# mx-mark/VideoTransformer-pytorch

Hardware: AMD Instinct MI355X
Metric: clips/sec TimeSformer-B divided_space_time 8x3x224x224 fwd+bwd (whole job) (higher is better)
Workload: dtype bf16

## Files before the change

videotransformer-pytorch_amd/csrc/gemm_nt.hip:

```cpp
#include "gemm_common.h"

namespace vtx {

constexpr int BK16 = 64;

__global__ __launch_bounds__(NT_THREADS) void gemm_nt_bf16_kernel(
    int M, int N, int K, const bf16raw* __restrict__ A, long lda, vtx_rowmap amap,
    const bf16raw* __restrict__ B, long ldb, int tiles_n, EpiParams ep) {
  extern __shared__ __attribute__((aligned(16))) char smem[];
  bf16raw* As = reinterpret_cast<bf16raw*>(smem);
  bf16raw* Bs = As + 2 * BM * BK16;
  const int tid = threadIdx.x, lane = tid & 63, wave = tid >> 6;
  const int wm = wave >> 1, wn = wave & 1;
  const int nwg = gridDim.x;
  const int tile = xcd_remap(blockIdx.x, nwg);
  const int tm = tile / tiles_n, tn = tile - tm * tiles_n;
  const int m0 = tm * BM, n0 = tn * BN;

  const int lc = tid & 7, lr = tid >> 3;
  const bf16raw* ap[4];
  const bf16raw* bp[4];
  int lds_off[4];
#pragma unroll
  for (int it = 0; it < 4; ++it) {
// ... 374 lines not shown
    asm volatile("" : "+v"(lq));
#pragma unroll
    for (int j = 0; j < 2; ++j) {
      const int rho = (wave * 2 + j) * 8 + (lq >> 3);
      const unsigned c2 = (unsigned)(((lq & 7) ^ ((rho >> 1) & 7)) * 16);
      const int la0 = min((rho >> 6) * 128 + (rho & 63), ml), la1 = min((rho >> 6) * 128 + (rho & 63) + 64, ml);
      const int lb0 = min((rho >> 5) * 64 + (rho & 31), nl), lb1 = min((rho >> 5) * 64 + (rho & 31) + 32, nl);
      unsigned ra0, ra1;
      if (CONT || am.fast) {
        ra0 = (unsigned)(la0 + (la0 >= bl ? am.skip : 0));
        ra1 = (unsigned)(la1 + (la1 >= bl ? am.skip : 0));
      } else {
        ra0 = (unsigned)(map_row(amap, m0s + la0) - first);
        ra1 = (unsigned)(map_row(amap, m0s + la1) - first);
      }
      off[0][j] = ra0 * lda2 + c2;
      off[3][j] = ra1 * lda2 + c2;
      off[1][j] = (unsigned)lb0 * ldb2 + c2;
      off[2][j] = (unsigned)lb1 * ldb2 + c2;
    }
  };
  auto issue = [&](int kind, int kt) {
    bf16raw* dst = lds + ((kt & 1) ^ par) * PP_BUF + kind * PP_REGION + wave * 1024;
    const char* base = ((kind == 0 || kind == 3) ? abase : bbase) + (long)kt * (PP_BK * 2);
    asm volatile("" : "+s"(base));
    dma16(reinterpret_cast<const bf16raw*>(base + off[kind][0]), dst);
    dma16(reinterpret_cast<const bf16raw*>(base + off[kind][1]), dst + 512);
  };
  auto prologue = [&]() {
    issue(0, 0); issue(1, 0); issue(2, 0); issue(3, 0);
    issue(0, 1); issue(1, 1); issue(2, 1);
  };

  const int l31 = lane & 31;
  int fr[4];
#pragma unroll
  for (int ks = 0; ks < 4; ++ks) fr[ks] = l31 * PP_BK + (((2 * ks + (lane >> 5)) ^ ((l31 >> 1) & 7)) << 3);
  const int a_grp = wr * 64 * PP_BK;
  const int b_grp = wc * 32 * PP_BK;

#define PP_READ_A(buf_, kind_)                                                                         \
  _Pragma("unroll") for (int i = 0; i < 2; ++i) _Pragma("unroll") for (int ks = 0; ks < 4; ++ks)       \
      fa[i][ks] = *reinterpret_cast<const bf16x8*>(lds + (buf_) * PP_BUF + (kind_) * PP_REGION + a_grp + i * 32 * PP_BK + fr[ks]);
#define PP_READ_B(buf_, kind_, fb_)                                                                    \
  _Pragma("unroll") for (int ks = 0; ks < 4; ++ks)                                                     \
      fb_[ks] = *reinterpret_cast<const bf16x8*>(lds + (buf_) * PP_BUF + (kind_) * PP_REGION + b_grp + fr[ks]);
#define PP_MMA(i0_, j_, fb_, ISSUE_) PP_MMA_H(i0_, j_, fb_, ISSUE_, , )
#ifndef VTX_PP_PRIO
#define VTX_PP_PRIO 1
#endif
#define PP_MMA_H(i0_, j_, fb_, ISSUE_, HW_, HB_)                                                       \
  if (VTX_PP_PRIO == 1) __builtin_amdgcn_s_setprio(1); else if (VTX_PP_PRIO == 3) __builtin_amdgcn_s_setprio(0); \
  _Pragma("unroll") for (int ks = 0; ks < 4; ++ks) {                                                   \
    _Pragma("unroll") for (int i = 0; i < 2; ++i)                                                      \
        acc[(i0_) + i][j_] = __builtin_amdgcn_mfma_f32_32x32x16_bf16(fa[i][ks], fb_[ks], acc[(i0_) + i][j_], 0, 0, 0); \
    if (ks == 0) { __builtin_amdgcn_sched_barrier(0); ISSUE_; HW_ __builtin_amdgcn_sched_barrier(0); HB_ }     \
  }                                                                                                    \
  if (VTX_PP_PRIO == 1) __builtin_amdgcn_s_setprio(0); else if (VTX_PP_PRIO == 3) __builtin_amdgcn_s_setprio(1);
#define PP_BAR() __builtin_amdgcn_s_barrier()

#ifndef VTX_PP_BF16_STAGE
#define VTX_PP_BF16_STAGE 1
#endif
#define PP_KTILE(E1_, E2_, W1_, W2_, W4_, ISS_, H1_, H2_, H3_, H4_) PP_KTILE_X(E1_, E2_, W1_, W2_, W4_, ISS_, H1_, H2_, H3_, H4_, false, false, false)
#define PP_KTILE_X(E1_, E2_, W1_, W2_, W4_, ISS_, H1_, H2_, H3_, H4_, X1_, X2_, X4_) \
    PP_KTILE_XH(E1_, E2_, W1_, W2_, W4_, ISS_, H1_, H2_, H3_, H4_, X1_, X2_, X4_, false, false, , , , )
#define PP_KTILE_XH(E1_, E2_, W1_, W2_, W4_, ISS_, H1_, H2_, H3_, H4_, X1_, X2_, X4_, X1R_, R4_, M3W_, M3B_, M4W_, M4B_) \
    {                                                                                                  \
      const int buf = (kt & 1) ^ par;                                                                  \
      const bool e1 = (E1_), e2 = (E2_);                   \
      const bool w1 = (W1_), w2 = (W2_);            \
                                                            \
      PP_READ_A(buf, 0);                                                                               \
      PP_READ_B(buf, 1, fb0);                                                                          \
      if (w1) { if (X1_) { if (X1R_) wait_vmcnt<8 + NST - NSR>(); else wait_vmcnt<8 + NST>(); } else wait_vmcnt<8>(); } else wait_vmcnt<2>(); \
      H1_                                                                                              \
      lgkm0();                                                                                         \
      PP_BAR();                                                                                        \
      PP_MMA(0, 0, fb0, ISS_(3, kt + 1, e1));                                                          \
      PP_BAR();                                                                                        \
                                                                \
      PP_READ_B(buf, 2, fb1);                                                                          \
      if (w1) { if (X2_) wait_vmcnt<8 + NST>(); else wait_vmcnt<8>(); } else wait_vmcnt<0>();          \
      H2_                                                                                              \
      lgkm0();                                                                                         \
      PP_BAR();                                                                                        \
      PP_MMA(0, 1, fb1, ISS_(0, kt + 2, e2));                                                          \
      PP_BAR();                                                                                        \
                                                                                     \
      PP_READ_A(buf, 3);                                                                               \
      H3_                                                                                              \
      lgkm0();                                                                                         \
      PP_BAR();                                                                                        \
      PP_MMA_H(2, 1, fb1, ISS_(1, kt + 2, e2), M3W_, M3B_);                                            \
      PP_BAR();                                                                                        \
                                 \
      if (W4_) { if (w2) { if (X4_) wait_vmcnt<8 + NST>(); else if (R4_) wait_vmcnt<10>(); else wait_vmcnt<8>(); } else if (w1) wait_vmcnt<4>(); } \
      H4_                                                                                              \
      PP_BAR();                                                                                        \
      PP_MMA_H(2, 0, fb0, ISS_(2, kt + 2, e2), M4W_, M4B_);                                            \
      PP_BAR();                                                                                        \
    }
#define PP_ISS_COND(kind_, ktv_, ex_) if (ex_) issue(kind_, ktv_)
#define PP_ISS_ALWAYS(kind_, ktv_, ex_) issue(kind_, ktv_)

  typedef __attribute__((address_space(3))) char lds_char;
  const unsigned slot_rd = (unsigned)(unsigned long)(lds_char*)(smem + PP_RING_BYTES);
  const unsigned bias_rd = (unsigned)(unsigned long)(lds_char*)(reinterpret_cast<char*>(stg) + 256 + (lane & 31) * 4);
  constexpr int NST = HAS_ACT ? 32 : 16;
  constexpr int NSR = NST / 4;
  bool relax = false;
  bool prev_rolled = false;
  int t = next_tile();
  const int tend = xcount;
  if (t >= tend) { check_out(); return; }
  int t_next = tend, t_nn = tend;
  if constexpr (CONT) t_next = next_tile();
  int pending = 0;
  if (EPI2 && !CONT && tid == 0) pending = atomicAdd(my_ctr, 1);
  set_tile(t, 0);
  m0 = m0s; n0 = n0s;
  prologue();
  while (true) {
    f32x16 acc[4][2];
#pragma unroll
    for (int i = 0; i < 4; ++i)
#pragma unroll
      for (int j = 0; j < 2; ++j)
#pragma unroll
        for (int r = 0; r < 16; ++r) acc[i][j][r] = 0.f;
    bf16x8 fa[2][4], fb0[4], fb1[4];
    if constexpr (PREG) {
      int lf = lane;
      asm volatile("" : "+v"(lf));
#pragma unroll
      for (int ks = 0; ks < 4; ++ks) fr[ks] = (lf & 31) * PP_BK + (((2 * ks + (lf >> 5)) ^ (((lf & 31) >> 1) & 7)) << 3);
    }
    const bool more_c = CONT && t_next < tend;
    const int em0 = m0 + wr * 128, en0 = n0 + wc * 64;
    const int tile_m0 = m0;
    TileMap cm;
    unsigned ldcb = 0, lean_skipb = 0;
    bool lean = false;
    [[maybe_unused]] bool rolled = false;
    int lean_lb = 0;
    const char* lean_cb = nullptr;
    [[maybe_unused]] __amdgpu_buffer_rsrc_t lean_rsrc;
    float bcol[2] = {0.f, 0.f};
    auto epi_head = [&]() {
      cm = make_tile_map(ep.cmap, tile_m0);
      ldcb = (unsigned)ep.ldc * 2u;
      const long skipb64 = (long)cm.skip * (long)ldcb;
      lean = CONT && (dbg == 0 || dbg == 5 || dbg == 6) && em0 + 127 < ep.M && en0 + 63 < ep.N && (ep.split_row <= 0 || em0 + 127 < ep.split_row) &&
             cm.fast && cm.skip >= 0 && skipb64 < (1L << 30) && ep.ldc < (1L << 22) && PRE != PRE_DGELU;
      if constexpr (HAS_ACT) lean = lean && ep.act == 2 && ep.ldc2 < (1L << 22);
      if constexpr (ROLL) lean = true;
      lean_lb = em0 < cm.bound ? cm.bound - em0 : 0x7fffffff;
      lean_cb = reinterpret_cast<const char*>(ep.C) + ((cm.base_q + em0 + (em0 >= cm.bound ? (long)cm.skip : 0L)) * ep.ldc + en0) * 2;
      lean_skipb = (unsigned)skipb64;
      if constexpr (ROLL) {
        const long last = (long)ep.cmap.base + (ep.M - 1) + (ep.cmap.grp > 0 ? (long)((unsigned)(ep.M - 1) / (unsigned)ep.cmap.grp) * ep.cmap.skip : 0L);
        const long left = en0 < ep.N ? (reinterpret_cast<const char*>(ep.C) + (last + 1) * ep.ldc * 2) - lean_cb : 0L;
        lean_rsrc = __builtin_amdgcn_make_buffer_rsrc(const_cast<char*>(lean_cb), 0, (int)(left < 0 ? 0 : (left > 0x7fffffffL ? 0x7fffffffL : left)), 0x00020000);
      }
    };
    typedef __attribute__((ext_vector_type(2))) __bf16 bf16x2;
    [[maybe_unused]] unsigned pl_wa0 = 0, pl_wa1 = 0, pl_rd = 0, pl_v0 = 0;
    [[maybe_unused]] int pl_p2 = 0;
    [[maybe_unused]] u32x4 pl_w0, pl_w1;
    auto pl_setup = [&]() {
      int ln = lane;
      asm volatile("" : "+v"(ln));
      const unsigned stg0 = (unsigned)(unsigned long)(lds_char*)(reinterpret_cast<char*>(stg));
      pl_p2 = ln >> 3;
      pl_wa0 = stg0 + (unsigned)(((ln >> 5) * 132 + (ln & 31)) * 4);
      pl_wa1 = pl_wa0 + 264 * 4;
      pl_rd = stg0 + (unsigned)((pl_p2 * 64 + 4 * ((pl_p2 >> 1) & 1) + 8 * (pl_p2 >> 2) + (ln & 7) * 8) * 4);
      pl_v0 = (unsigned)(2 * pl_p2) * ldcb + (unsigned)(ln & 7) * 16u;
    };
#define PP_LWAIT(n_, ...) asm volatile("s_waitcnt lgkmcnt(%[cnt])" : __VA_ARGS__ : [cnt] "n"(n_) : "memory"); __builtin_amdgcn_sched_barrier(0)
#define PP_PWAIT(n_) PP_LWAIT(n_, "+v"(pl_w0), "+v"(pl_w1))
#define PP_PW(mi_, half_) if (ep.bias) { PP_PW_(mi_, half_, true) } else { PP_PW_(mi_, half_, false) }
#define PP_PW_(mi_, half_, B_)                                                                          \
    {                                                                                                   \
      _Pragma("unroll") for (int kk = 0; kk < 2; ++kk) _Pragma("unroll") for (int ni = 0; ni < 2; ++ni) { \
        f32x2 lo = mk2(acc[mi_][ni][8 * (half_) + 4 * kk], acc[mi_][ni][8 * (half_) + 4 * kk + 1]);     \
        f32x2 hi = mk2(acc[mi_][ni][8 * (half_) + 4 * kk + 2], acc[mi_][ni][8 * (half_) + 4 * kk + 3]); \
        if (B_) { const f32x2 b2 = mk2(bcol[ni], bcol[ni]); lo = lo + b2; hi = hi + b2; }               \
        union { bf16x2 v; unsigned u; } x;      \
        union { bf16x2 v; unsigned u; } y;      \
        x.v[0] = (__bf16)lo[0]; x.v[1] = (__bf16)lo[1];                                                 \
        y.v[0] = (__bf16)hi[0]; y.v[1] = (__bf16)hi[1];                                                 \
        if (ni == 0) asm volatile("ds_write2_b32 %0, %1, %2 offset1:64" :: "v"(kk ? pl_wa1 : pl_wa0), "v"(x.u), "v"(y.u) : "memory"); \
        else asm volatile("ds_write2_b32 %0, %1, %2 offset0:32 offset1:96" :: "v"(kk ? pl_wa1 : pl_wa0), "v"(x.u), "v"(y.u) : "memory"); \
      }                                                                                                 \
    }
#define PP_PR() asm volatile("ds_read_b128 %0, %2\n\tds_read_b128 %1, %2 offset:16" : "=&v"(pl_w0), "=&v"(pl_w1) : "v"(pl_rd) : "memory")
#define PP_PF(p_)                                                                                       \
    {                                                                                                   \
      const char* base = lean_cb + (long)(16 * (p_)) * ldcb;                                            \
      if constexpr (!ROLL) asm volatile("" : "+s"(base));            \
      _Pragma("unroll") for (int u = 0; u < 2; ++u) {                                                   \
        const unsigned sel = u ? 0x07060302u : 0x05040100u;                                             \
        u32x4 o;                                                                                        \
        o[0] = __builtin_amdgcn_perm(pl_w0[1], pl_w0[0], sel);                                          \
        o[1] = __builtin_amdgcn_perm(pl_w0[3], pl_w0[2], sel);                                          \
        o[2] = __builtin_amdgcn_perm(pl_w1[1], pl_w1[0], sel);                                          \
        o[3] = __builtin_amdgcn_perm(pl_w1[3], pl_w1[2], sel);                                          \
        const unsigned voff = pl_v0 + (u ? ldcb : 0u) + ((2 * pl_p2 + u >= lean_lb - 16 * (p_)) ? lean_skipb : 0u); \
         \
         \
        if constexpr (ROLL) __builtin_amdgcn_raw_buffer_store_b128(o, lean_rsrc, voff + (unsigned)(16 * (p_)) * ldcb, 0, 2); \
        else st16_nt_b(base, voff, o);                                                                  \
      }                                                                                                 \
    }
    constexpr bool ROLLK = ROLL;
    static_assert(!ROLL || (CONT && VTX_PP_BF16_STAGE && PRE == PRE_NONE && !HAS_SC && !HAS_ACT), "rolling: the plain continuous flow only");
    stamp(0);
    if (relax) wait_vmcnt<10 + NST>(); else wait_vmcnt<10>();
    PP_BAR();
    stamp(1);
    if (wr == 1) PP_BAR();
    if constexpr (CONT) {
      auto bias_dma = [&]() {
        if (ep.bias) {
          const int c = n0 + wc * 64 + lane;
          __builtin_amdgcn_global_load_lds((const __attribute__((address_space(1))) void*)(ep.bias + (c < ep.N ? c : 0)),
// ... 10 lines not shown
            const int idx = split ? (ml - ep.split_row) : (int)q1 * ep.rs_m1 + (ml - (int)q2 * ep.rs_d2) * ep.rs_m2;
            __builtin_amdgcn_global_load_lds((const __attribute__((address_space(1))) void*)(ep.row_scale + idx),
                                             (__attribute__((address_space(3))) void*)(stg + 128 + h * 64), 4, 0, 0);
          }
        }
      };
      int drawn;
      asm volatile("" : "=v"(drawn));
      const int one = 1;
      int kt = 0;
      if (more_c) {
#define PP_CF_H1 if (kt == 0) bias_dma();                                                                        \
                 if (kt == 1 && tid == 0)                                                                        \
                   asm volatile("global_atomic_add %0, %1, %2, off sc0" : "=&v"(drawn) : "v"(my_ctr), "v"(one) : "memory");
#define PP_CF_H2 if (kt == nk - 2) set_tile(t_next, (long)nk * (PP_BK * 2));
#define PP_CF_H3 if (kt == 2) {                                                                                  \
                   int v;                                                                                        \
                   asm volatile("ds_read_b32 %0, %1\n\ts_waitcnt lgkmcnt(0)" : "=&v"(v) : "v"(slot_rd) : "memory"); \
                   t_nn = __builtin_amdgcn_readfirstlane(v);                                                     \
                 }
#define PP_CF_H4 if (kt == 1 && wave == 0) {                                                                     \
                   wait_vmcnt<6>();                                                                              \
                   if (tid == 0) asm volatile("ds_write_b32 %0, %1" :: "v"(slot_rd), "v"(drawn) : "memory");     \
                   lgkm0();                                                                                      \
                 }
        for (; kt < nk - 1; ++kt) {
          PP_KTILE_XH(true, true, true, true, true, PP_ISS_ALWAYS, PP_CF_H1, PP_CF_H2;, PP_CF_H3, PP_CF_H4,
                      relax && kt < 2, relax && kt == 0, relax && kt == 0, prev_rolled && kt == 1, false, , , , )
        }
        if constexpr (ROLLK) {
          epi_head();
          rolled = true;
          const bool full = em0 + 127 < ep.M && en0 + 63 < ep.N && trace == nullptr;
          if (ep.bias) asm volatile("ds_read_b32 %0, %2\n\tds_read_b32 %1, %2 offset:128\n\ts_waitcnt lgkmcnt(0)"
                                    : "=&v"(bcol[0]), "=&v"(bcol[1]) : "v"(bias_rd) : "memory");
          pl_setup();
          PP_KTILE_XH(true, true, true, true, true, PP_ISS_ALWAYS, , , PP_PW(0, 0) PP_PR();,
                      PP_PWAIT(0); PP_PF(1) PP_PW(1, 0) PP_PR();,
                      false, false, false, false, full,
                      , PP_PF(0) PP_PW(0, 1) PP_PR();,
                      PP_PWAIT(0);, PP_PF(2) PP_PW(1, 1) PP_PR();)
        } else {
          PP_KTILE_XH(true, true, true, true, true, PP_ISS_ALWAYS, PP_CF_H1, PP_CF_H2;, PP_CF_H3, PP_CF_H4,
                      relax && kt < 2, relax && kt == 0, relax && kt == 0, prev_rolled && kt == 1, false, , , , )
        }
#undef PP_CF_H1
#undef PP_CF_H2
#undef PP_CF_H3
#undef PP_CF_H4
      } else {
        for (; kt < nk; ++kt) {
          PP_KTILE(kt + 1 < nk, kt + 2 < nk, kt + 1 < nk, kt + 2 < nk, true, PP_ISS_COND, if (kt == 0) bias_dma();, , , )
        }
      }
    } else {
      for (int kt = 0; kt < nk; ++kt) {
        PP_KTILE(kt + 1 < nk, kt + 2 < nk, kt + 1 < nk, kt + 2 < nk, true, PP_ISS_COND, , , , )
      }
    }
    if (wr == 0) PP_BAR();
    stamp(2);
    if constexpr (!EPI2) {
      t = next_tile();
      const bool more = t < tend;
      if (more) { set_tile(t, 0); m0 = m0s; n0 = n0s; prologue(); }
#define PP_EPI(mi_, half_)                                                                              \
      {                                                                                                 \
        const int col = lane & 31, rhalf = (lane >> 5) * 4;                                             \
        _Pragma("unroll") for (int ni = 0; ni < 2; ++ni) _Pragma("unroll") for (int r = 0; r < 8; ++r)  \
            stg[((r & 3) + 8 * (r >> 2) + rhalf) * PP_STG_LD + ni * 32 + col] = acc[mi_][ni][8 * (half_) + r]; \
        lgkm0();                                                                                        \
        __builtin_amdgcn_wave_barrier();                                                                \
        epilogue<bf16raw, 16, 2, PP_STG_LD>(ep, stg, em0 + (mi_) * 32 + (half_) * 16, en0, lane);       \
        lgkm0();                                                                                        \
        __builtin_amdgcn_wave_barrier();                                                                \
      }
      PP_EPI(0, 0) PP_EPI(0, 1) PP_EPI(1, 0) PP_EPI(1, 1) PP_EPI(2, 0) PP_EPI(2, 1) PP_EPI(3, 0) PP_EPI(3, 1)
#undef PP_EPI
      if (!more) break;
    } else {
      bool more = more_c;
      if constexpr (!CONT) {
        t = publish(pending);
        more = t < tend;
      }
      stamp(3);
      int le = lane;
      asm volatile("" : "+v"(le));
      const int en = en0 + (le & 7) * 8;
      const bool col_ok = en < ep.N;
      const int enc = col_ok ? en : 0;
      const int er = em0 + (le >> 3);
      constexpr bool HAS_PRE = PRE != PRE_NONE, pre_res = PRE == PRE_RES;
      bf16raw* const pre_lds = lds + wave * (128 * 64);
      if (!rolled) epi_head();
      [[maybe_unused]] u32x4 blk[16];
      auto blk_load = [&]() {
        const unsigned penc2 = col_ok ? (unsigned)en * 2u : 0u;
        const unsigned pld2 = (unsigned)(pre_res ? ep.ldr : ep.ld_dgelu) * 2u;
        const int lastv = min(ep.M - 1, (pre_res && ep.split_row > 0) ? ep.split_row - 1 : 0x7fffffff);
        const int m0c = min(tile_m0, lastv);
        const TileMap prm = make_tile_map(ep.rmap, m0c);
        const long pfirst = pre_res ? tile_map_row_u(prm, ep.rmap, m0c) : (long)m0c;
// ... 4 lines not shown
        const int plast = lastv - m0c;
        const int pl0 = (tile_m0 - m0c) + wr * 128 + (le >> 3);
#pragma unroll
        for (int j = 0; j < 16; ++j) {
          const int l = min(pl0 + 8 * j, plast);
          const int lr = l + (l >= pbl ? pskip : 0);
          const unsigned vo = (unsigned)lr * pld2 + penc2;
          asm volatile("global_load_dwordx4 %0, %1, %2 nt" : "=v"(blk[j]) : "v"(vo), "s"(pbase) : "memory");
        }
      };
#define PP_BLOAD() if constexpr (PREG) blk_load()
#define PP_BLK(p_, u_) (PREG ? blk[2 * (p_) + (u_)] : pre[u_])
#define PP_BWAIT(p_) if constexpr (PREG) { asm volatile("s_waitcnt vmcnt(%2)" : "+v"(blk[2 * (p_)]), "+v"(blk[2 * (p_) + 1]) : "n"(14 - 2 * (p_)) : "memory"); }
      if constexpr (HAS_PRE && !CONT) {
        const bf16raw* const pre_base = reinterpret_cast<const bf16raw*>(pre_res ? ep.R : ep.dgelu_in);
        const long pre_ld = pre_res ? ep.ldr : ep.ld_dgelu;
        const TileMap rm = make_tile_map(ep.rmap, tile_m0);
        const int row_last = ep.M - 1;
#pragma unroll
        for (int j = 0; j < 16; ++j) {
          int ml = er + 8 * j;
          const bool past = ml > row_last;
          if (past) ml = row_last;
          long rr = ml;
          if (pre_res) {
            const bool split = ep.split_row > 0 && ml >= ep.split_row;
            rr = split ? 0 : (ep.r_period > 0 ? (long)(ml % ep.r_period) : (past ? map_row(ep.rmap, ml) : tile_map_row(rm, ep.rmap, ml)));
          }
          dma16(pre_base + rr * pre_ld + enc, pre_lds + j * 512);
        }
      }
      if (ep.bias && !rolled) {
        if constexpr (CONT) {
          asm volatile("ds_read_b32 %0, %2\n\tds_read_b32 %1, %2 offset:128\n\ts_waitcnt lgkmcnt(0)"
                       : "=&v"(bcol[0]), "=&v"(bcol[1]) : "v"(bias_rd) : "memory");
        } else {
#pragma unroll
          for (int ni = 0; ni < 2; ++ni) {
            const int c = en0 + ni * 32 + (le & 31);
            bcol[ni] = ep.bias[c < ep.N ? c : 0];
          }
        }
      }
      float sc[8][2];
      float scl[2] = {0.f, 0.f};
      if constexpr (HAS_SC && CONT) {
        if (lean || PREG) {
          const unsigned scl_rd = (unsigned)(unsigned long)(lds_char*)(reinterpret_cast<char*>(stg) + 512 + le * 4);
          asm volatile("ds_read_b32 %0, %2\n\tds_read_b32 %1, %2 offset:256\n\ts_waitcnt lgkmcnt(0)"
                       : "=&v"(scl[0]), "=&v"(scl[1]) : "v"(scl_rd) : "memory");
        } else {
        const unsigned sc_rd = (unsigned)(unsigned long)(lds_char*)(reinterpret_cast<char*>(stg) + 512 + (le >> 3) * 4);
        asm volatile("ds_read_b32 %0, %16\n\tds_read_b32 %1, %16 offset:32\n\tds_read_b32 %2, %16 offset:64\n\t"
                     "ds_read_b32 %3, %16 offset:96\n\tds_read_b32 %4, %16 offset:128\n\tds_read_b32 %5, %16 offset:160\n\t"
                     "ds_read_b32 %6, %16 offset:192\n\tds_read_b32 %7, %16 offset:224\n\tds_read_b32 %8, %16 offset:256\n\t"
                     "ds_read_b32 %9, %16 offset:288\n\tds_read_b32 %10, %16 offset:320\n\tds_read_b32 %11, %16 offset:352\n\t"
                     "ds_read_b32 %12, %16 offset:384\n\tds_read_b32 %13, %16 offset:416\n\tds_read_b32 %14, %16 offset:448\n\t"
                     "ds_read_b32 %15, %16 offset:480\n\ts_waitcnt lgkmcnt(0)"
                     : "=&v"(sc[0][0]), "=&v"(sc[0][1]), "=&v"(sc[1][0]), "=&v"(sc[1][1]), "=&v"(sc[2][0]), "=&v"(sc[2][1]),
                       "=&v"(sc[3][0]), "=&v"(sc[3][1]), "=&v"(sc[4][0]), "=&v"(sc[4][1]), "=&v"(sc[5][0]), "=&v"(sc[5][1]),
                       "=&v"(sc[6][0]), "=&v"(sc[6][1]), "=&v"(sc[7][0]), "=&v"(sc[7][1])
                     : "v"(sc_rd) : "memory");
        }
      }
      if constexpr (HAS_SC && !CONT) {
        auto scale_of = [&](int ml) -> float {
          if (ml >= ep.M) ml = ep.M - 1;
          const bool split = ep.split_row > 0 && ml >= ep.split_row;
          const unsigned q1 = fast_div((unsigned)ml, ep.rs_magic1, ep.rs_shift1);
          const unsigned q2 = fast_div((unsigned)ml, ep.rs_magic2, ep.rs_shift2);
          return ep.row_scale[split ? (ml - ep.split_row) : (int)q1 * ep.rs_m1 + (ml - (int)q2 * ep.rs_d2) * ep.rs_m2];
        };
        if (lean) {
          scl[0] = scale_of(em0 + le);
          scl[1] = scale_of(em0 + 64 + le);
        } else {
#pragma unroll
          for (int p = 0; p < 8; ++p)
#pragma unroll
            for (int u = 0; u < 2; ++u) sc[p][u] = scale_of(er + 16 * p + 8 * u);
        }
      }
      if constexpr (!CONT) {
        if (more && tid == 0) pending = atomicAdd(my_ctr, 1);
        asm volatile("s_waitcnt vmcnt(0)" ::: "memory");
        stamp(4);
        asm volatile("" : "+v"(bcol[0]));
        asm volatile("" : "+v"(bcol[1]));
        if constexpr (HAS_SC) {
#pragma unroll
          for (int p = 0; p < 8; ++p) { asm volatile("" : "+v"(sc[p][0])); asm volatile("" : "+v"(sc[p][1])); }
          asm volatile("" : "+v"(scl[0])); asm volatile("" : "+v"(scl[1]));
        }
        if constexpr (!HAS_PRE) {
          if (more) { set_tile(t, 0); m0 = m0s; n0 = n0s; prologue(); }
        }
      }
      stamp(5);
      const unsigned stg_rd = (unsigned)(unsigned long)(lds_char*)(reinterpret_cast<char*>(stg) +
                                                                    ((le >> 3) * PP_STG_LD + (le & 7) * 8) * 4);
      const unsigned pre_rd = (unsigned)(unsigned long)(lds_char*)(reinterpret_cast<char*>(pre_lds) + le * 16);
      const int kpar = nk & 1;
#define PP_EPI2(p_, mi_, half_)                                                                         \
      {                                                                                                 \
         \
         \
        int lp = le;                                                                                    \
        if constexpr (PREG) asm volatile("" : "+v"(lp));                                                \
        const int enp = PREG ? en0 + (lp & 7) * 8 : en, erp = PREG ? em0 + (lp >> 3) : er;              \
        const bool cokp = PREG ? enp < ep.N : col_ok;                                                   \
        const int col = lp & 31, rhalf = (lp >> 5) * 4;                                                 \
        if (dbg != 3) {                                                                                 \
        _Pragma("unroll") for (int ni = 0; ni < 2; ++ni) _Pragma("unroll") for (int r = 0; r < 8; ++r)  \
            stg[((r & 3) + 8 * (r >> 2) + rhalf) * PP_STG_LD + ni * 32 + col] = acc[mi_][ni][8 * (half_) + r] + bcol[ni]; \
        } else { stg[lp] = acc[mi_][0][8 * (half_)] + acc[mi_][1][8 * (half_) + 7]; }                 \
        lgkm0();                                                                                        \
        __builtin_amdgcn_wave_barrier();                                                                \
        f32x4 s00, s01, s10, s11;                                                                       \
        u32x4 pre[2];                                                                                   \
        PP_BWAIT(p_)                                                                                    \
        [[maybe_unused]] float scp[2];                \
        if constexpr (HAS_SC && PREG)                                                                   \
          asm volatile("ds_bpermute_b32 %0, %2, %3 offset:%4\n\tds_bpermute_b32 %1, %2, %3 offset:%5\n\ts_waitcnt lgkmcnt(0)" \
                       : "=&v"(scp[0]), "=&v"(scp[1]) : "v"((unsigned)(lp >> 3) * 4u), "v"((p_) < 4 ? scl[0] : scl[1]), \
                         "n"(((16 * (p_)) & 63) * 4), "n"(((16 * (p_) + 8) & 63) * 4) : "memory");     \
        if constexpr (HAS_PRE && !PREG) {                                                               \
          const unsigned prd__ = pre_rd + 2 * (p_) * 1024;                                              \
          asm volatile("ds_read_b128 %0, %6\n\tds_read_b128 %1, %6 offset:16\n\t"                       \
                       "ds_read_b128 %2, %6 offset:2048\n\tds_read_b128 %3, %6 offset:2064\n\t"         \
                       "ds_read_b128 %4, %7\n\tds_read_b128 %5, %7 offset:1024\n\t"                     \
                       "s_waitcnt lgkmcnt(0)"                                                           \
                       : "=&v"(s00), "=&v"(s01), "=&v"(s10), "=&v"(s11), "=&v"(pre[0]), "=&v"(pre[1])   \
                       : "v"(stg_rd), "v"(prd__) : "memory");                                           \
        } else                                                                                            \
          asm volatile("ds_read_b128 %0, %4\n\tds_read_b128 %1, %4 offset:16\n\t"                       \
                       "ds_read_b128 %2, %4 offset:2048\n\tds_read_b128 %3, %4 offset:2064\n\t"         \
                       "s_waitcnt lgkmcnt(0)"                                                           \
                       : "=&v"(s00), "=&v"(s01), "=&v"(s10), "=&v"(s11) : "v"(stg_rd) : "memory");      \
        __builtin_amdgcn_sched_barrier(0);                                                              \
        float v[2][8];                                                                                  \
        _Pragma("unroll") for (int j = 0; j < 4; ++j) {                                                 \
          v[0][j] = s00[j]; v[0][4 + j] = s01[j]; v[1][j] = s10[j]; v[1][4 + j] = s11[j];               \
        }                                                                                               \
        _Pragma("unroll") for (int u = 0; u < 2; ++u) {                                                 \
          const int m = erp + 16 * (p_) + 8 * u;                                                        \
          const bool ok = cokp && m < ep.M && dbg != 2;                                                 \
          const bool split = ep.split_row > 0 && m >= ep.split_row;                                     \
          if constexpr (HAS_ACT) {                                                                      \
// ... 27 lines not shown
            _Pragma("unroll") for (int j = 0; j < 4; ++j) {                                             \
              v[u][2 * j] += __uint_as_float(w[j] << 16);                                               \
              v[u][2 * j + 1] += __uint_as_float(w[j] & 0xffff0000u);                                   \
            }                                                                                           \
          }                                                                                             \
          if (ok) {                                                                                     \
            if (split) store8(reinterpret_cast<bf16raw*>(ep.Csplit) + (long)(m - ep.split_row) * ep.ldsplit + enp, v[u]); \
            else PP_ST8(reinterpret_cast<bf16raw*>(ep.C) + tile_map_row(cm, ep.cmap, m) * ep.ldc + enp, v[u]); \
          }                                                                                             \
        }                                                                                               \
      }
      constexpr bool PAIRS = VTX_PP_BF16_STAGE && PRE == PRE_NONE && !HAS_SC && !HAS_ACT;
      const unsigned stg_wr0 = (unsigned)(unsigned long)(lds_char*)(reinterpret_cast<char*>(stg)) ;
      if (lean) {
        int ln = le;
        asm volatile("" : "+v"(ln));
        if constexpr (PAIRS) {
          if (rolled) {
            PP_PWAIT(0); PP_PF(3)
          } else {
            pl_setup();
            PP_PW(0, 0) PP_PR();
            PP_PW(0, 1) PP_PWAIT(4); PP_PF(0) PP_PR();
            PP_PW(1, 0) PP_PWAIT(4); PP_PF(1) PP_PR();
            PP_PW(1, 1) PP_PWAIT(4); PP_PF(2) PP_PR();
            PP_PWAIT(0); PP_PF(3)
          }
          PP_PW(2, 0) PP_PR();
          PP_PW(2, 1) PP_PWAIT(4); PP_PF(4) PP_PR();
          PP_PW(3, 0) PP_PWAIT(4); PP_PF(5) PP_PR();
          PP_PW(3, 1) PP_PWAIT(4); PP_PF(6) PP_PR();
          PP_PWAIT(0); PP_PF(7)
        } else {
          const unsigned wa0 = stg_wr0 + (unsigned)(((ln >> 5) * 256 + (ln & 31)) * 4), wa1 = wa0 + 512 * 4;
          const unsigned vf0 = (unsigned)(ln >> 3) * ldcb + (unsigned)(ln & 7) * 16u;
          const unsigned ldc2b = (unsigned)ep.ldc2 * 2u;
          const unsigned vg0 = (unsigned)(ln >> 3) * ldc2b + (unsigned)(ln & 7) * 16u;
          const char* const lean_c2b = reinterpret_cast<const char*>(ep.C2) + ((long)em0 * ep.ldc2 + en0) * 2;
          f32x4 s00, s01, s10, s11;
          u32x4 pre[2];
          float scu[2] = {1.f, 1.f};
          const unsigned bp_addr = (unsigned)(ln >> 3) * 4u;
          PP_BLOAD();
#define PP_LW(mi_, half_) if (ep.bias) { PP_LW_(mi_, half_, true) } else { PP_LW_(mi_, half_, false) }
#define PP_LW_(mi_, half_, B_)                                                                          \
          {                                                                                             \
            _Pragma("unroll") for (int kk = 0; kk < 2; ++kk) _Pragma("unroll") for (int ni = 0; ni < 2; ++ni) \
            _Pragma("unroll") for (int r2 = 0; r2 < 2; ++r2) {                                          \
              f32x2 xy = mk2(acc[mi_][ni][8 * (half_) + 4 * kk + 2 * r2], acc[mi_][ni][8 * (half_) + 4 * kk + 2 * r2 + 1]); \
              if (B_) { const f32x2 b2 = mk2(bcol[ni], bcol[ni]); xy = xy + b2; }                       \
              const float x = xy[0];                                                                    \
              const float y = xy[1];                                                                    \
              const unsigned wa = kk ? wa1 : wa0;                                                       \
              if (ni == 0 && r2 == 0) asm volatile("ds_write2_b32 %0, %1, %2 offset1:64" :: "v"(wa), "v"(x), "v"(y) : "memory"); \
              if (ni == 0 && r2 == 1) asm volatile("ds_write2_b32 %0, %1, %2 offset0:128 offset1:192" :: "v"(wa), "v"(x), "v"(y) : "memory"); \
              if (ni == 1 && r2 == 0) asm volatile("ds_write2_b32 %0, %1, %2 offset0:32 offset1:96" :: "v"(wa), "v"(x), "v"(y) : "memory"); \
              if (ni == 1 && r2 == 1) asm volatile("ds_write2_b32 %0, %1, %2 offset0:160 offset1:224" :: "v"(wa), "v"(x), "v"(y) : "memory"); \
            }                                                                                           \
          }
#define PP_LR(p_)                                                                                       \
          if constexpr (HAS_PRE && !PREG) {                                                             \
            const unsigned prd__ = pre_rd + 2 * (p_) * 1024;                                            \
            asm volatile("ds_read_b128 %0, %6\n\tds_read_b128 %1, %6 offset:16\n\t"                     \
                         "ds_read_b128 %2, %6 offset:2048\n\tds_read_b128 %3, %6 offset:2064\n\t"       \
                         "ds_read_b128 %4, %7\n\tds_read_b128 %5, %7 offset:1024"                       \
                         : "=&v"(s00), "=&v"(s01), "=&v"(s10), "=&v"(s11), "=&v"(pre[0]), "=&v"(pre[1]) \
                         : "v"(stg_rd), "v"(prd__) : "memory");                                         \
          } else                                                                                        \
            asm volatile("ds_read_b128 %0, %4\n\tds_read_b128 %1, %4 offset:16\n\t"                     \
                         "ds_read_b128 %2, %4 offset:2048\n\tds_read_b128 %3, %4 offset:2064"           \
                         : "=&v"(s00), "=&v"(s01), "=&v"(s10), "=&v"(s11) : "v"(stg_rd) : "memory");      \
          if constexpr (HAS_SC)                         \
            asm volatile("ds_bpermute_b32 %0, %2, %3 offset:%4\n\tds_bpermute_b32 %1, %2, %3 offset:%5"   \
                         : "=&v"(scu[0]), "=&v"(scu[1]) : "v"(bp_addr), "v"((p_) < 4 ? scl[0] : scl[1]),   \
                           "n"(((16 * (p_)) & 63) * 4), "n"(((16 * (p_) + 8) & 63) * 4) : "memory")
#define PP_LWAITF(n_)                                                                                   \
          if constexpr (HAS_PRE && !PREG) { PP_LWAIT(n_, "+v"(s00), "+v"(s01), "+v"(s10), "+v"(s11), "+v"(pre[0]), "+v"(pre[1]), "+v"(scu[0]), "+v"(scu[1])); } \
          else { PP_LWAIT(n_, "+v"(s00), "+v"(s01), "+v"(s10), "+v"(s11), "+v"(scu[0]), "+v"(scu[1])); }
#define PP_LF(p_)                                                                                       \
          {                                                                                             \
            _Pragma("clang fp contract(off)")         \
            PP_BWAIT(p_)                              \
            float v[2][8];                                                                              \
            _Pragma("unroll") for (int j = 0; j < 4; ++j) {                                             \
              v[0][j] = s00[j]; v[0][4 + j] = s01[j]; v[1][j] = s10[j]; v[1][4 + j] = s11[j];           \
            }                                                                                           \
            const char* const base = lean_cb + (long)(16 * (p_)) * ldcb;                                \
            _Pragma("unroll") for (int u = 0; u < 2; ++u) {                                             \
              if constexpr (HAS_ACT) {                       \
                float gp[8];                                                                            \
// ... 9 lines not shown
              }                                                                                         \
              if constexpr (HAS_SC) { _Pragma("unroll") for (int j = 0; j < 8; ++j) v[u][j] *= scu[u]; } \
              if constexpr (pre_res) {                               \
                const u32x4 w = PP_BLK(p_, u);                                                          \
                _Pragma("unroll") for (int j = 0; j < 4; ++j) {                                         \
                  v[u][2 * j] += __uint_as_float(w[j] << 16);                                           \
                  v[u][2 * j + 1] += __uint_as_float(w[j] & 0xffff0000u);                               \
                }                                                                                       \
              }                                                                                         \
              const unsigned voff = vf0 + (u ? 8u * ldcb : 0u) +                                        \
                                    (((ln >> 3) + 8 * u >= lean_lb - 16 * (p_)) ? lean_skipb : 0u);   \
              st16_nt_s(base, voff, pack8(v[u]));                                                       \
            }                                                                                           \
          }
          PP_LW(0, 0) PP_LR(0);
          PP_LW(0, 1) PP_LWAITF(8) PP_LF(0) PP_LR(1);
          PP_LW(1, 0) PP_LWAITF(8) PP_LF(1) PP_LR(2);
          PP_LW(1, 1) PP_LWAITF(8) PP_LF(2) PP_LR(3);
          PP_LW(2, 0) PP_LWAITF(8) PP_LF(3) PP_LR(4);
          PP_LW(2, 1) PP_LWAITF(8) PP_LF(4) PP_LR(5);
          PP_LW(3, 0) PP_LWAITF(8) PP_LF(5) PP_LR(6);
          PP_LW(3, 1) PP_LWAITF(8) PP_LF(6) PP_LR(7);
          PP_LWAITF(0) PP_LF(7)
#undef PP_LW
#undef PP_LW_
#undef PP_LR
#undef PP_LWAITF
#undef PP_LF
        }
      } else if constexpr (PAIRS) {
        unsigned* const stgw = reinterpret_cast<unsigned*>(stg);
        const int p2 = le >> 3;
        const unsigned pair_rd = (unsigned)(unsigned long)(lds_char*)(reinterpret_cast<char*>(stg) +
                                                                       (p2 * 64 + 4 * ((p2 >> 1) & 1) + 8 * (p2 >> 2) + (le & 7) * 8) * 4);
        typedef __attribute__((ext_vector_type(2))) __bf16 bf16x2;
#define PP_EPI2B(p_, mi_, half_)                                                                        \
        {                                                                                               \
          const int col = le & 31, hi = le >> 5;                                                    \
          _Pragma("unroll") for (int ni = 0; ni < 2; ++ni) _Pragma("unroll") for (int k = 0; k < 4; ++k) { \
                 \
            const int rp = ((2 * k) & 3) / 2 + 4 * ((2 * k) >> 2) + 2 * hi;                             \
            union { bf16x2 v; unsigned u; } w;                                                          \
            w.v[0] = (__bf16)(acc[mi_][ni][8 * (half_) + 2 * k] + bcol[ni]);                            \
            w.v[1] = (__bf16)(acc[mi_][ni][8 * (half_) + 2 * k + 1] + bcol[ni]);                        \
            stgw[rp * 64 + 4 * ((rp >> 1) & 1) + 8 * (rp >> 2) + ni * 32 + col] = w.u;                  \
          }                                                                                             \
          lgkm0();                                                                                      \
          __builtin_amdgcn_wave_barrier();                                                              \
          u32x4 w0, w1;                                                                                 \
          asm volatile("ds_read_b128 %0, %2\n\tds_read_b128 %1, %2 offset:16\n\ts_waitcnt lgkmcnt(0)"  \
                       : "=&v"(w0), "=&v"(w1) : "v"(pair_rd) : "memory");                               \
          __builtin_amdgcn_sched_barrier(0);                                                            \
          _Pragma("unroll") for (int u = 0; u < 2; ++u) {                                               \
            const unsigned sel = u ? 0x07060302u : 0x05040100u;     \
            u32x4 o;                                                                                    \
            o[0] = __builtin_amdgcn_perm(w0[1], w0[0], sel);                                            \
            o[1] = __builtin_amdgcn_perm(w0[3], w0[2], sel);                                            \
            o[2] = __builtin_amdgcn_perm(w1[1], w1[0], sel);                                            \
            o[3] = __builtin_amdgcn_perm(w1[3], w1[2], sel);                                            \
            const int m = em0 + 16 * (p_) + 2 * p2 + u;                                                 \
            const bool ok = col_ok && m < ep.M && dbg != 2;                                             \
            const bool split = ep.split_row > 0 && m >= ep.split_row;                                   \
            if (ok) {                                                                                   \
              if (split) *reinterpret_cast<u32x4*>(reinterpret_cast<bf16raw*>(ep.Csplit) + (long)(m - ep.split_row) * ep.ldsplit + en) = o; \
              else __builtin_nontemporal_store(o, reinterpret_cast<u32x4*>(reinterpret_cast<bf16raw*>(ep.C) + tile_map_row(cm, ep.cmap, m) * ep.ldc + en)); \
            }                                                                                           \
          }                                                                                             \
          __builtin_amdgcn_wave_barrier();                                                              \
        }
        PP_EPI2B(0, 0, 0) PP_EPI2B(1, 0, 1) PP_EPI2B(2, 1, 0) PP_EPI2B(3, 1, 1)
        PP_EPI2B(4, 2, 0) PP_EPI2B(5, 2, 1) PP_EPI2B(6, 3, 0) PP_EPI2B(7, 3, 1)
#undef PP_EPI2B
      } else {
        PP_BLOAD();
        PP_EPI2(0, 0, 0) PP_EPI2(1, 0, 1) PP_EPI2(2, 1, 0) PP_EPI2(3, 1, 1)
        PP_EPI2(4, 2, 0) PP_EPI2(5, 2, 1) PP_EPI2(6, 3, 0) PP_EPI2(7, 3, 1)
      }
#undef PP_EPI2
// ... 257 lines not shown
```

Baseline: 765.1.

## Switch ping-pong GEMM from 32x32x16 to 16x16x32 MFMA tiles

Replaces the 32x32x16 bf16 MFMA with 16x16x32 MFMA in the ping-pong NT GEMM kernel. The accumulator layout, LDS fragment reads, bias loading and every epilogue staging path are rewritten to match, with new XOR swizzles to avoid bank conflicts. The 16x16 instruction has different throughput and latency characteristics and a smaller per-lane accumulator footprint, but it needs more instructions per tile and a more intricate epilogue addressing scheme, which risks both correctness and register pressure.

```diff
diff --git a/videotransformer-pytorch_amd/csrc/gemm_nt.hip b/videotransformer-pytorch_amd/csrc/gemm_nt.hip
--- a/videotransformer-pytorch_amd/csrc/gemm_nt.hip
+++ b/videotransformer-pytorch_amd/csrc/gemm_nt.hip
@@ -430,29 +430,32 @@
     issue(0, 1); issue(1, 1); issue(2, 1);
   };
 
-  const int l31 = lane & 31;
-  int fr[4];
-#pragma unroll
-  for (int ks = 0; ks < 4; ++ks) fr[ks] = l31 * PP_BK + (((2 * ks + (lane >> 5)) ^ ((l31 >> 1) & 7)) << 3);
+  const int l15 = lane & 15;
+  int fr[2];
+#pragma unroll
+  for (int ks = 0; ks < 2; ++ks) fr[ks] = l15 * PP_BK + (((4 * ks + (lane >> 4)) ^ ((l15 >> 1) & 7)) << 3);
   const int a_grp = wr * 64 * PP_BK;
   const int b_grp = wc * 32 * PP_BK;
 
 #define PP_READ_A(buf_, kind_)                                                                         \
-  _Pragma("unroll") for (int i = 0; i < 2; ++i) _Pragma("unroll") for (int ks = 0; ks < 4; ++ks)       \
-      fa[i][ks] = *reinterpret_cast<const bf16x8*>(lds + (buf_) * PP_BUF + (kind_) * PP_REGION + a_grp + i * 32 * PP_BK + fr[ks]);
+  _Pragma("unroll") for (int i = 0; i < 2; ++i) _Pragma("unroll") for (int q = 0; q < 4; ++q)          \
+      fa[2 * i + (q >> 1)][q & 1] = *reinterpret_cast<const bf16x8*>(lds + (buf_) * PP_BUF + (kind_) * PP_REGION + a_grp + (i * 32 + (q >> 1) * 16) * PP_BK + fr[q & 1]);
 #define PP_READ_B(buf_, kind_, fb_)                                                                    \
-  _Pragma("unroll") for (int ks = 0; ks < 4; ++ks)                                                     \
-      fb_[ks] = *reinterpret_cast<const bf16x8*>(lds + (buf_) * PP_BUF + (kind_) * PP_REGION + b_grp + fr[ks]);
+  _Pragma("unroll") for (int q = 0; q < 4; ++q)                                                        \
+      fb_[q >> 1][q & 1] = *reinterpret_cast<const bf16x8*>(lds + (buf_) * PP_BUF + (kind_) * PP_REGION + b_grp + (q >> 1) * 16 * PP_BK + fr[q & 1]);
 #define PP_MMA(i0_, j_, fb_, ISSUE_) PP_MMA_H(i0_, j_, fb_, ISSUE_, , )
 #ifndef VTX_PP_PRIO
 #define VTX_PP_PRIO 1
 #endif
 #define PP_MMA_H(i0_, j_, fb_, ISSUE_, HW_, HB_)                                                       \
   if (VTX_PP_PRIO == 1) __builtin_amdgcn_s_setprio(1); else if (VTX_PP_PRIO == 3) __builtin_amdgcn_s_setprio(0); \
-  _Pragma("unroll") for (int ks = 0; ks < 4; ++ks) {                                                   \
-    _Pragma("unroll") for (int i = 0; i < 2; ++i)                                                      \
-        acc[(i0_) + i][j_] = __builtin_amdgcn_mfma_f32_32x32x16_bf16(fa[i][ks], fb_[ks], acc[(i0_) + i][j_], 0, 0, 0); \
-    if (ks == 0) { __builtin_amdgcn_sched_barrier(0); ISSUE_; HW_ __builtin_amdgcn_sched_barrier(0); HB_ }     \
+  _Pragma("unroll") for (int ks = 0; ks < 2; ++ks) {                                                   \
+    _Pragma("unroll") for (int i = 0; i < 2; ++i) {                                                    \
+      _Pragma("unroll") for (int q = 0; q < 4; ++q)                                                    \
+        acc[4 * (i0_) + 2 * i + (q >> 1)][2 * (j_) + (q & 1)] = __builtin_amdgcn_mfma_f32_16x16x32_bf16(   \
+            fa[2 * i + (q >> 1)][ks], fb_[q & 1][ks], acc[4 * (i0_) + 2 * i + (q >> 1)][2 * (j_) + (q & 1)], 0, 0, 0); \
+      if (ks == 0 && i == 0) { __builtin_amdgcn_sched_barrier(0); ISSUE_; HW_ __builtin_amdgcn_sched_barrier(0); HB_ } \
+    }                                                                                                  \
   }                                                                                                    \
   if (VTX_PP_PRIO == 1) __builtin_amdgcn_s_setprio(0); else if (VTX_PP_PRIO == 3) __builtin_amdgcn_s_setprio(1);
 #define PP_BAR() __builtin_amdgcn_s_barrier()
@@ -490,13 +493,13 @@
       H3_                                                                                              \
       lgkm0();                                                                                         \
       PP_BAR();                                                                                        \
-      PP_MMA_H(2, 1, fb1, ISS_(1, kt + 2, e2), M3W_, M3B_);                                            \
+      PP_MMA_H(1, 1, fb1, ISS_(1, kt + 2, e2), M3W_, M3B_);                                            \
       PP_BAR();                                                                                        \
                                  \
       if (W4_) { if (w2) { if (X4_) wait_vmcnt<8 + NST>(); else if (R4_) wait_vmcnt<10>(); else wait_vmcnt<8>(); } else if (w1) wait_vmcnt<4>(); } \
       H4_                                                                                              \
       PP_BAR();                                                                                        \
-      PP_MMA_H(2, 0, fb0, ISS_(2, kt + 2, e2), M4W_, M4B_);                                            \
+      PP_MMA_H(1, 0, fb0, ISS_(2, kt + 2, e2), M4W_, M4B_);                                            \
       PP_BAR();                                                                                        \
     }
 #define PP_ISS_COND(kind_, ktv_, ex_) if (ex_) issue(kind_, ktv_)
@@ -504,7 +507,7 @@
 
   typedef __attribute__((address_space(3))) char lds_char;
   const unsigned slot_rd = (unsigned)(unsigned long)(lds_char*)(smem + PP_RING_BYTES);
-  const unsigned bias_rd = (unsigned)(unsigned long)(lds_char*)(reinterpret_cast<char*>(stg) + 256 + (lane & 31) * 4);
+  const unsigned bias_rd = (unsigned)(unsigned long)(lds_char*)(reinterpret_cast<char*>(stg) + 256 + (lane & 15) * 4);
   constexpr int NST = HAS_ACT ? 32 : 16;
   constexpr int NSR = NST / 4;
   bool relax = false;
@@ -520,19 +523,19 @@
   m0 = m0s; n0 = n0s;
   prologue();
   while (true) {
-    f32x16 acc[4][2];
-#pragma unroll
-    for (int i = 0; i < 4; ++i)
-#pragma unroll
-      for (int j = 0; j < 2; ++j)
-#pragma unroll
-        for (int r = 0; r < 16; ++r) acc[i][j][r] = 0.f;
-    bf16x8 fa[2][4], fb0[4], fb1[4];
+    f32x4 acc[8][4];
+#pragma unroll
+    for (int i = 0; i < 8; ++i)
+#pragma unroll
+      for (int j = 0; j < 4; ++j)
+#pragma unroll
+        for (int r = 0; r < 4; ++r) acc[i][j][r] = 0.f;
+    bf16x8 fa[4][2], fb0[2][2], fb1[2][2];
     if constexpr (PREG) {
       int lf = lane;
       asm volatile("" : "+v"(lf));
 #pragma unroll
-      for (int ks = 0; ks < 4; ++ks) fr[ks] = (lf & 31) * PP_BK + (((2 * ks + (lf >> 5)) ^ (((lf & 31) >> 1) & 7)) << 3);
+      for (int ks = 0; ks < 2; ++ks) fr[ks] = (lf & 15) * PP_BK + (((4 * ks + (lf >> 4)) ^ (((lf & 15) >> 1) & 7)) << 3);
     }
     const bool more_c = CONT && t_next < tend;
     const int em0 = m0 + wr * 128, en0 = n0 + wc * 64;
@@ -544,7 +547,7 @@
     int lean_lb = 0;
     const char* lean_cb = nullptr;
     [[maybe_unused]] __amdgpu_buffer_rsrc_t lean_rsrc;
-    float bcol[2] = {0.f, 0.f};
+    float bcol[4] = {0.f, 0.f, 0.f, 0.f};
     auto epi_head = [&]() {
       cm = make_tile_map(ep.cmap, tile_m0);
       ldcb = (unsigned)ep.ldc * 2u;
@@ -571,26 +574,28 @@
       asm volatile("" : "+v"(ln));
       const unsigned stg0 = (unsigned)(unsigned long)(lds_char*)(reinterpret_cast<char*>(stg));
       pl_p2 = ln >> 3;
-      pl_wa0 = stg0 + (unsigned)(((ln >> 5) * 132 + (ln & 31)) * 4);
-      pl_wa1 = pl_wa0 + 264 * 4;
-      pl_rd = stg0 + (unsigned)((pl_p2 * 64 + 4 * ((pl_p2 >> 1) & 1) + 8 * (pl_p2 >> 2) + (ln & 7) * 8) * 4);
+      pl_wa0 = stg0 + (unsigned)(((ln >> 4) * 192 + (ln & 15) + 16 * ((ln >> 4) & 1)) * 4);
+      pl_wa1 = stg0 + (unsigned)(((ln >> 4) * 192 + (ln & 15) - 16 * ((ln >> 4) & 1)) * 4);
+      pl_rd = stg0 + (unsigned)(((pl_p2 >> 1) * 192 + (pl_p2 & 1) * 68 + ((ln & 7) ^ (2 * ((pl_p2 >> 1) & 1))) * 8) * 4);
       pl_v0 = (unsigned)(2 * pl_p2) * ldcb + (unsigned)(ln & 7) * 16u;
     };
 #define PP_LWAIT(n_, ...) asm volatile("s_waitcnt lgkmcnt(%[cnt])" : __VA_ARGS__ : [cnt] "n"(n_) : "memory"); __builtin_amdgcn_sched_barrier(0)
 #define PP_PWAIT(n_) PP_LWAIT(n_, "+v"(pl_w0), "+v"(pl_w1))
-#define PP_PW(mi_, half_) if (ep.bias) { PP_PW_(mi_, half_, true) } else { PP_PW_(mi_, half_, false) }
-#define PP_PW_(mi_, half_, B_)                                                                          \
+#define PP_PW(mi_, half_) if (ep.bias) { PP_PW_(2 * (mi_) + (half_), true) } else { PP_PW_(2 * (mi_) + (half_), false) }
+#define PP_PW_(p_, B_)                                                                                  \
     {                                                                                                   \
-      _Pragma("unroll") for (int kk = 0; kk < 2; ++kk) _Pragma("unroll") for (int ni = 0; ni < 2; ++ni) { \
-        f32x2 lo = mk2(acc[mi_][ni][8 * (half_) + 4 * kk], acc[mi_][ni][8 * (half_) + 4 * kk + 1]);     \
-        f32x2 hi = mk2(acc[mi_][ni][8 * (half_) + 4 * kk + 2], acc[mi_][ni][8 * (half_) + 4 * kk + 3]); \
+      _Pragma("unroll") for (int ni = 0; ni < 4; ++ni) {                                                \
+        f32x2 lo = mk2(acc[p_][ni][0], acc[p_][ni][1]);                                                 \
+        f32x2 hi = mk2(acc[p_][ni][2], acc[p_][ni][3]);                                                 \
         if (B_) { const f32x2 b2 = mk2(bcol[ni], bcol[ni]); lo = lo + b2; hi = hi + b2; }               \
         union { bf16x2 v; unsigned u; } x;      \
         union { bf16x2 v; unsigned u; } y;      \
         x.v[0] = (__bf16)lo[0]; x.v[1] = (__bf16)lo[1];                                                 \
         y.v[0] = (__bf16)hi[0]; y.v[1] = (__bf16)hi[1];                                                 \
-        if (ni == 0) asm volatile("ds_write2_b32 %0, %1, %2 offset1:64" :: "v"(kk ? pl_wa1 : pl_wa0), "v"(x.u), "v"(y.u) : "memory"); \
-        else asm volatile("ds_write2_b32 %0, %1, %2 offset0:32 offset1:96" :: "v"(kk ? pl_wa1 : pl_wa0), "v"(x.u), "v"(y.u) : "memory"); \
+        if (ni == 0) asm volatile("ds_write2_b32 %0, %1, %2 offset1:68" :: "v"(pl_wa0), "v"(x.u), "v"(y.u) : "memory"); \
+        if (ni == 1) asm volatile("ds_write2_b32 %0, %1, %2 offset0:16 offset1:84" :: "v"(pl_wa1), "v"(x.u), "v"(y.u) : "memory"); \
+        if (ni == 2) asm volatile("ds_write2_b32 %0, %1, %2 offset0:32 offset1:100" :: "v"(pl_wa0), "v"(x.u), "v"(y.u) : "memory"); \
+        if (ni == 3) asm volatile("ds_write2_b32 %0, %1, %2 offset0:48 offset1:116" :: "v"(pl_wa1), "v"(x.u), "v"(y.u) : "memory"); \
       }                                                                                                 \
     }
 #define PP_PR() asm volatile("ds_read_b128 %0, %2\n\tds_read_b128 %1, %2 offset:16" : "=&v"(pl_w0), "=&v"(pl_w1) : "v"(pl_rd) : "memory")
@@ -667,8 +672,8 @@
           epi_head();
           rolled = true;
           const bool full = em0 + 127 < ep.M && en0 + 63 < ep.N && trace == nullptr;
-          if (ep.bias) asm volatile("ds_read_b32 %0, %2\n\tds_read_b32 %1, %2 offset:128\n\ts_waitcnt lgkmcnt(0)"
-                                    : "=&v"(bcol[0]), "=&v"(bcol[1]) : "v"(bias_rd) : "memory");
+          if (ep.bias) asm volatile("ds_read_b32 %0, %4\n\tds_read_b32 %1, %4 offset:64\n\tds_read_b32 %2, %4 offset:128\n\tds_read_b32 %3, %4 offset:192\n\ts_waitcnt lgkmcnt(0)"
+                                    : "=&v"(bcol[0]), "=&v"(bcol[1]), "=&v"(bcol[2]), "=&v"(bcol[3]) : "v"(bias_rd) : "memory");
           pl_setup();
           PP_KTILE_XH(true, true, true, true, true, PP_ISS_ALWAYS, , , PP_PW(0, 0) PP_PR();,
                       PP_PWAIT(0); PP_PF(1) PP_PW(1, 0) PP_PR();,
@@ -701,9 +706,9 @@
       if (more) { set_tile(t, 0); m0 = m0s; n0 = n0s; prologue(); }
 #define PP_EPI(mi_, half_)                                                                              \
       {                                                                                                 \
-        const int col = lane & 31, rhalf = (lane >> 5) * 4;                                             \
-        _Pragma("unroll") for (int ni = 0; ni < 2; ++ni) _Pragma("unroll") for (int r = 0; r < 8; ++r)  \
-            stg[((r & 3) + 8 * (r >> 2) + rhalf) * PP_STG_LD + ni * 32 + col] = acc[mi_][ni][8 * (half_) + r]; \
+        const int col = lane & 15, r0 = (lane >> 4) * 4;                                                \
+        _Pragma("unroll") for (int ni = 0; ni < 4; ++ni) _Pragma("unroll") for (int r = 0; r < 4; ++r)  \
+            stg[(r0 + r) * PP_STG_LD + ni * 16 + col] = acc[2 * (mi_) + (half_)][ni][r];                \
         lgkm0();                                                                                        \
         __builtin_amdgcn_wave_barrier();                                                                \
         epilogue<bf16raw, 16, 2, PP_STG_LD>(ep, stg, em0 + (mi_) * 32 + (half_) * 16, en0, lane);       \
@@ -774,12 +779,12 @@
       }
       if (ep.bias && !rolled) {
         if constexpr (CONT) {
-          asm volatile("ds_read_b32 %0, %2\n\tds_read_b32 %1, %2 offset:128\n\ts_waitcnt lgkmcnt(0)"
-                       : "=&v"(bcol[0]), "=&v"(bcol[1]) : "v"(bias_rd) : "memory");
+          asm volatile("ds_read_b32 %0, %4\n\tds_read_b32 %1, %4 offset:64\n\tds_read_b32 %2, %4 offset:128\n\tds_read_b32 %3, %4 offset:192\n\ts_waitcnt lgkmcnt(0)"
+                       : "=&v"(bcol[0]), "=&v"(bcol[1]), "=&v"(bcol[2]), "=&v"(bcol[3]) : "v"(bias_rd) : "memory");
         } else {
 #pragma unroll
-          for (int ni = 0; ni < 2; ++ni) {
-            const int c = en0 + ni * 32 + (le & 31);
+          for (int ni = 0; ni < 4; ++ni) {
+            const int c = en0 + ni * 16 + (le & 15);
             bcol[ni] = ep.bias[c < ep.N ? c : 0];
           }
         }
@@ -829,6 +834,8 @@
         stamp(4);
         asm volatile("" : "+v"(bcol[0]));
         asm volatile("" : "+v"(bcol[1]));
+        asm volatile("" : "+v"(bcol[2]));
+        asm volatile("" : "+v"(bcol[3]));
         if constexpr (HAS_SC) {
 #pragma unroll
           for (int p = 0; p < 8; ++p) { asm volatile("" : "+v"(sc[p][0])); asm volatile("" : "+v"(sc[p][1])); }
@@ -840,7 +847,7 @@
       }
       stamp(5);
       const unsigned stg_rd = (unsigned)(unsigned long)(lds_char*)(reinterpret_cast<char*>(stg) +
-                                                                    ((le >> 3) * PP_STG_LD + (le & 7) * 8) * 4);
+                                                                    ((le >> 3) * PP_STG_LD + ((le & 7) ^ (((le >> 5) & 1) * 2)) * 8) * 4);
       const unsigned pre_rd = (unsigned)(unsigned long)(lds_char*)(reinterpret_cast<char*>(pre_lds) + le * 16);
       const int kpar = nk & 1;
 #define PP_EPI2(p_, mi_, half_)                                                                         \
@@ -851,11 +858,11 @@
         if constexpr (PREG) asm volatile("" : "+v"(lp));                                                \
         const int enp = PREG ? en0 + (lp & 7) * 8 : en, erp = PREG ? em0 + (lp >> 3) : er;              \
         const bool cokp = PREG ? enp < ep.N : col_ok;                                                   \
-        const int col = lp & 31, rhalf = (lp >> 5) * 4;                                                 \
+        const int col = lp & 15, r0 = (lp >> 4) * 4, sw = ((lp >> 4) & 1) * 16;                         \
         if (dbg != 3) {                                                                                 \
-        _Pragma("unroll") for (int ni = 0; ni < 2; ++ni) _Pragma("unroll") for (int r = 0; r < 8; ++r)  \
-            stg[((r & 3) + 8 * (r >> 2) + rhalf) * PP_STG_LD + ni * 32 + col] = acc[mi_][ni][8 * (half_) + r] + bcol[ni]; \
-        } else { stg[lp] = acc[mi_][0][8 * (half_)] + acc[mi_][1][8 * (half_) + 7]; }                 \
+        _Pragma("unroll") for (int ni = 0; ni < 4; ++ni) _Pragma("unroll") for (int r = 0; r < 4; ++r)  \
+            stg[(r0 + r) * PP_STG_LD + ((ni * 16 + col) ^ sw)] = acc[p_][ni][r] + bcol[ni];             \
+        } else { stg[lp] = acc[p_][0][0] + acc[p_][3][3]; }                                             \
         lgkm0();                                                                                        \
         __builtin_amdgcn_wave_barrier();                                                                \
         f32x4 s00, s01, s10, s11;                                                                       \
@@ -949,7 +956,8 @@
           PP_PW(3, 1) PP_PWAIT(4); PP_PF(6) PP_PR();
           PP_PWAIT(0); PP_PF(7)
         } else {
-          const unsigned wa0 = stg_wr0 + (unsigned)(((ln >> 5) * 256 + (ln & 31)) * 4), wa1 = wa0 + 512 * 4;
+          const unsigned wa0 = stg_wr0 + (unsigned)(((ln >> 4) * 256 + (ln & 15) + 16 * ((ln >> 4) & 1)) * 4);
+          const unsigned wa1 = stg_wr0 + (unsigned)(((ln >> 4) * 256 + (ln & 15) - 16 * ((ln >> 4) & 1)) * 4);
           const unsigned vf0 = (unsigned)(ln >> 3) * ldcb + (unsigned)(ln & 7) * 16u;
           const unsigned ldc2b = (unsigned)ep.ldc2 * 2u;
           const unsigned vg0 = (unsigned)(ln >> 3) * ldc2b + (unsigned)(ln & 7) * 16u;
@@ -959,20 +967,23 @@
           float scu[2] = {1.f, 1.f};
           const unsigned bp_addr = (unsigned)(ln >> 3) * 4u;
           PP_BLOAD();
-#define PP_LW(mi_, half_) if (ep.bias) { PP_LW_(mi_, half_, true) } else { PP_LW_(mi_, half_, false) }
-#define PP_LW_(mi_, half_, B_)                                                                          \
+#define PP_LW(mi_, half_) if (ep.bias) { PP_LW_(2 * (mi_) + (half_), true) } else { PP_LW_(2 * (mi_) + (half_), false) }
+#define PP_LW_(p_, B_)                                                                                  \
           {                                                                                             \
-            _Pragma("unroll") for (int kk = 0; kk < 2; ++kk) _Pragma("unroll") for (int ni = 0; ni < 2; ++ni) \
-            _Pragma("unroll") for (int r2 = 0; r2 < 2; ++r2) {                                          \
-              f32x2 xy = mk2(acc[mi_][ni][8 * (half_) + 4 * kk + 2 * r2], acc[mi_][ni][8 * (half_) + 4 * kk + 2 * r2 + 1]); \
+            _Pragma("unroll") for (int ni = 0; ni < 4; ++ni) _Pragma("unroll") for (int r2 = 0; r2 < 2; ++r2) { \
+              f32x2 xy = mk2(acc[p_][ni][2 * r2], acc[p_][ni][2 * r2 + 1]);                             \
               if (B_) { const f32x2 b2 = mk2(bcol[ni], bcol[ni]); xy = xy + b2; }                       \
               const float x = xy[0];                                                                    \
               const float y = xy[1];                                                                    \
-              const unsigned wa = kk ? wa1 : wa0;                                                       \
+              const unsigned wa = (ni & 1) ? wa1 : wa0;                                                 \
               if (ni == 0 && r2 == 0) asm volatile("ds_write2_b32 %0, %1, %2 offset1:64" :: "v"(wa), "v"(x), "v"(y) : "memory"); \
               if (ni == 0 && r2 == 1) asm volatile("ds_write2_b32 %0, %1, %2 offset0:128 offset1:192" :: "v"(wa), "v"(x), "v"(y) : "memory"); \
-              if (ni == 1 && r2 == 0) asm volatile("ds_write2_b32 %0, %1, %2 offset0:32 offset1:96" :: "v"(wa), "v"(x), "v"(y) : "memory"); \
-              if (ni == 1 && r2 == 1) asm volatile("ds_write2_b32 %0, %1, %2 offset0:160 offset1:224" :: "v"(wa), "v"(x), "v"(y) : "memory"); \
+              if (ni == 1 && r2 == 0) asm volatile("ds_write2_b32 %0, %1, %2 offset0:16 offset1:80" :: "v"(wa), "v"(x), "v"(y) : "memory"); \
+              if (ni == 1 && r2 == 1) asm volatile("ds_write2_b32 %0, %1, %2 offset0:144 offset1:208" :: "v"(wa), "v"(x), "v"(y) : "memory"); \
+              if (ni == 2 && r2 == 0) asm volatile("ds_write2_b32 %0, %1, %2 offset0:32 offset1:96" :: "v"(wa), "v"(x), "v"(y) : "memory"); \
+              if (ni == 2 && r2 == 1) asm volatile("ds_write2_b32 %0, %1, %2 offset0:160 offset1:224" :: "v"(wa), "v"(x), "v"(y) : "memory"); \
+              if (ni == 3 && r2 == 0) asm volatile("ds_write2_b32 %0, %1, %2 offset0:48 offset1:112" :: "v"(wa), "v"(x), "v"(y) : "memory"); \
+              if (ni == 3 && r2 == 1) asm volatile("ds_write2_b32 %0, %1, %2 offset0:176 offset1:240" :: "v"(wa), "v"(x), "v"(y) : "memory"); \
             }                                                                                           \
           }
 #define PP_LR(p_)                                                                                       \
@@ -1048,18 +1059,17 @@
         unsigned* const stgw = reinterpret_cast<unsigned*>(stg);
         const int p2 = le >> 3;
         const unsigned pair_rd = (unsigned)(unsigned long)(lds_char*)(reinterpret_cast<char*>(stg) +
-                                                                       (p2 * 64 + 4 * ((p2 >> 1) & 1) + 8 * (p2 >> 2) + (le & 7) * 8) * 4);
+                                                                       ((p2 >> 1) * 192 + (p2 & 1) * 68 + ((le & 7) ^ (2 * ((p2 >> 1) & 1))) * 8) * 4);
         typedef __attribute__((ext_vector_type(2))) __bf16 bf16x2;
 #define PP_EPI2B(p_, mi_, half_)                                                                        \
         {                                                                                               \
-          const int col = le & 31, hi = le >> 5;                                                    \
-          _Pragma("unroll") for (int ni = 0; ni < 2; ++ni) _Pragma("unroll") for (int k = 0; k < 4; ++k) { \
-                 \
-            const int rp = ((2 * k) & 3) / 2 + 4 * ((2 * k) >> 2) + 2 * hi;                             \
+          const int col = le & 15, g = le >> 4;                                                         \
+          _Pragma("unroll") for (int ni = 0; ni < 4; ++ni) _Pragma("unroll") for (int k = 0; k < 2; ++k) { \
+                       \
             union { bf16x2 v; unsigned u; } w;                                                          \
-            w.v[0] = (__bf16)(acc[mi_][ni][8 * (half_) + 2 * k] + bcol[ni]);                            \
-            w.v[1] = (__bf16)(acc[mi_][ni][8 * (half_) + 2 * k + 1] + bcol[ni]);                        \
-            stgw[rp * 64 + 4 * ((rp >> 1) & 1) + 8 * (rp >> 2) + ni * 32 + col] = w.u;                  \
+            w.v[0] = (__bf16)(acc[p_][ni][2 * k] + bcol[ni]);                                           \
+            w.v[1] = (__bf16)(acc[p_][ni][2 * k + 1] + bcol[ni]);                                       \
+            stgw[g * 192 + k * 68 + ((ni * 16 + col) ^ (16 * (g & 1)))] = w.u;                          \
           }                                                                                             \
           lgkm0();                                                                                      \
           __builtin_amdgcn_wave_barrier();                                                              \
```

After: 783.2, median of 6. 2.4% higher.
